# jianhengLiu/VINS-RGBD-FAST

Hardware: AMD Instinct MI355X
Metric: VIO frames/sec (640x480, 150 feats, 10-KF window) (higher is better)
Workload: dtype f64; 1 GPU; BASELINE configs[2]: 128 independent synthetic 640x480 RGB-D + 200 Hz IMU sequences per MI355X, 150 features, 10-keyframe window; sequences_per_gpu=128, tracker_lag=1, parallelism=sequences sharded per GPU, no data-path collective

## Files before the change

### vins-rgbd-fast_amd/csrc/be_kernels.hip

```cpp
#include <hip/hip_runtime.h>
#include "kernels.h"
#include "be_factors.h"

using namespace dm;

#if VIO_TIMERS
#define PH_INIT long long ph_t0 = (s == 0 && threadIdx.x == 0) ? VIO_CLOCK() : 0
#define PH(k) do { if (s == 0 && threadIdx.x == 0) { long long n_ = VIO_CLOCK(); B.timings[k] += (float)(n_ - ph_t0); ph_t0 = n_; } } while (0)
#else
#define PH_INIT do {} while (0)
#define PH(k) do {} while (0)
#endif

namespace {

struct Ctx {
    float *timings;
    const DevCfg *C;
    int s, W, P, LW, NL, NLs, NPR;
    BeSeq *be;
    FeSeq *fe;
    const vio_calibration *K;
    PreInt *pre;
    int *lm_id, *lm_start, *lm_nobs, *lm_est, *lm_solve, *lm_dyn, *lm_order, *lm_free, *lm_tmp, *lm_pidx, *lm_aidx, *lm_relo;
// ... 209 lines not shown
__device__ void lm_compact(Ctx &c, int *flags, int *offs, int *scratch) {
    int n = c.be->n_lm;
    int kept = block_scan_flags(flags, n, offs, scratch);
    const int t = threadIdx.x, nt = blockDim.x;
    int nfree0 = c.be->n_free;
    for (int k = t; k < n; k += nt) c.lm_tmp[k] = c.lm_order[k];
    __syncthreads();
    for (int k = t; k < n; k += nt) {
        int slot = c.lm_tmp[k];
        if (flags[k]) c.lm_order[offs[k]] = slot;
        else c.lm_free[nfree0 + (k - offs[k])] = slot;
    }
    __syncthreads();
    if (t == 0) { c.be->n_lm = kept; c.be->n_free = nfree0 + (n - kept); }
    __syncthreads();
}

}

__device__ m3 pnp_rodrigues(v3 r) {
    const double th = nrm(r);
    if (th < 2.220446049250313e-16) return eye();
    const v3 k = scl(1.0 / th, r);
    const double cth = cos(th), sth = sin(th), c1 = 1 - cth;
    const m3 K = skew(k);
    const double kk[3] = {k.x, k.y, k.z};
    m3 R;
    for (int i = 0; i < 3; i++) for (int j = 0; j < 3; j++) R.a[i * 3 + j] = (i == j ? cth : 0.0) + c1 * kk[i] * kk[j] + sth * K.a[i * 3 + j];
    return R;
}
// ... 1308 lines not shown
                be.initFirstPoseFlag = 0; be.prevTime = -1; be.n_lm = 0; be.n_free = c.NL; be.ring_base = 0;
                be.imu_head = be.imu_count_ingest;
                be.relo_info = 0;
                be.reboot_count++;
                be.status_code = VIO_REBOOTED;
                be.rebooted = 1;
                be.do_marg = 0;
                be.overflow = 0;
            }
        }
    }
}

}

template <bool EXACT> __device__ void marg_body(const Batch &B, int s, int *scratch, double *sred, unsigned char *smem_marg);
__device__ void finish_body(const Batch &B, int s, int *scratch, PreWork &pw, unsigned char *smem_marg);

__device__ __forceinline__ void solve_body(const Batch &B, int s, int *scratch, double *sred, unsigned char *smem, PreWork &pw);

__global__ __launch_bounds__(1024) void be_solve_kernel(Batch B) {
    const int s = blockIdx.x + B.s0;
    __shared__ int scratch[2 * 1024 + 8];
    __shared__ double sred[64];
    extern __shared__ __attribute__((aligned(16))) unsigned char smem[];
    PreWork &pw = *(PreWork *)(smem + 16 * ((B.cfg->LW * 8 + 15) / 16));
    solve_body(B, s, scratch, sred, smem, pw);
}
__global__ __launch_bounds__(512) void be_solve_kernel_512(Batch B) {
    const int s = blockIdx.x + B.s0;
    __shared__ int scratch[2 * 1024 + 8];
    __shared__ double sred[64];
    extern __shared__ __attribute__((aligned(16))) unsigned char smem[];
    PreWork &pw = *(PreWork *)(smem + 16 * ((B.cfg->LW * 8 + 15) / 16));
    solve_body(B, s, scratch, sred, smem, pw);
}
__global__ __launch_bounds__(512) void be_marg_kernel(Batch B) {
    const int s = blockIdx.x + B.s0;
    __shared__ int scratch[2 * 512 + 8];
    __shared__ double sred[64];
    __shared__ PreWork pw;
    extern __shared__ __attribute__((aligned(16))) unsigned char smem[];
    marg_body<false>(B, s, scratch, sred, smem);
    __syncthreads();
    finish_body(B, s, scratch, pw, smem);
}
__global__ __launch_bounds__(512) void be_marg_exact_kernel(Batch B) {
    const int s = blockIdx.x + B.s0;
    __shared__ int scratch[2 * 512 + 8];
    __shared__ double sred[64];
    __shared__ PreWork pw;
    extern __shared__ __attribute__((aligned(16))) unsigned char smem[];
    marg_body<true>(B, s, scratch, sred, smem);
    __syncthreads();
    finish_body(B, s, scratch, pw, smem);
}

__device__ __forceinline__ void solve_body(const Batch &B, int s, int *scratch, double *sred, unsigned char *smem, PreWork &pw) {
    const int t = threadIdx.x, nt = blockDim.x;
    Ctx c = make_ctx(B, s);
    const DevCfg &C = *B.cfg;
    const vio_config &cfg = C.c;
    BeSeq &be = *c.be;
    if (!be.do_solve) return;
    const int W = c.W, P = c.P, LW = c.LW, W1 = W + 1;
    __shared__ Params X, Xc;
    __shared__ double sdx[6 * VIO_MAXW + 16], srp[6 * VIO_MAXW + 16];
    __shared__ int sh_i[8];
    __shared__ double sh_d[8];
    double *xs = (double *)smem;
// ... 467 lines not shown
    }
    for (int i = t; i < n; i += nt) {
        double sacc = b[md + i];
        for (int k = 0; k < md; k++) sacc -= ET1[(size_t)i * m + k] * b[k];
        for (int k = md; k < m; k++) sacc -= ET1[(size_t)i * m + k] * c.gl[k - md];
        br[i] = sacc;
    }
    __syncthreads();
    if (VIO_TIMERS && t == 0) be.dbg[8] = (int)(VIO_CLOCK() - tx0);
    const int sw2 = marg_literal_prior(c, be, Ar, br, n, c.margW, A, sred, smem);
    if (VIO_TIMERS && t == 0) be.dbg[9] = (int)(VIO_CLOCK() - tx0);
    if (t == 0) { be.dbg[0] = sw1 * 100 + sw2; be.dbg[2] = second_new ? 1 : 0; be.dbg[4] = m; }
    if (VIO_TIMERS && t == 0) be.dbg[10] = (int)(VIO_CLOCK() - tx0);
}

template <bool EXACT> __device__ void marg_body(const Batch &B, int s, int *scratch, double *sred, unsigned char *smem_marg) {
    const int t = threadIdx.x, nt = blockDim.x;
    Ctx c = make_ctx(B, s);
    const DevCfg &C = *B.cfg;
    const vio_config &cfg = C.c;
    BeSeq &be = *c.be;
    if (!be.do_marg || be.rebooted || be.frame_count < c.W) return;
    const int W = c.W, W1 = W + 1, n = c.NPR;
    const double eps = 1e-8;
    __shared__ Params X;
    __shared__ double sdx[6 * VIO_MAXW + 16], srp[6 * VIO_MAXW + 16];
    __shared__ double cs[VIO_MAXW * 3 + 10], sn[VIO_MAXW * 3 + 10];
    __shared__ int pp[VIO_MAXW * 3 + 10], qq[VIO_MAXW * 3 + 10];
    __shared__ double A15[225], V15[225], Pinv[225];
    __shared__ int newpresent[VIO_MAXW + 3];
    const bool second_new = be.marginalization_flag != 0;
// ... 10 lines not shown
        quat q = R2q(ldm(be.Rs[i]));
        X.pose[i * 7 + 3] = q.x; X.pose[i * 7 + 4] = q.y; X.pose[i * 7 + 5] = q.z; X.pose[i * 7 + 6] = q.w;
        for (int k = 0; k < 3; k++) { X.sb[i * 9 + k] = be.Vs[i][k]; X.sb[i * 9 + 3 + k] = be.Bas[i][k]; X.sb[i * 9 + 6 + k] = be.Bgs[i][k]; }
    }
    if (t == W + 1) {
        X.ex[0] = be.tic[0]; X.ex[1] = be.tic[1]; X.ex[2] = be.tic[2];
        quat q = R2q(ldm(be.ric));
        X.ex[3] = q.x; X.ex[4] = q.y; X.ex[5] = q.z; X.ex[6] = q.w;
        X.td = be.td;
    }
    if (t < W + 3) newpresent[t] = 0;
    __syncthreads();
    if (t <= W) for (int k = 0; k < 7; k++) be.para_Pose[t][k] = X.pose[t * 7 + k];
    const int md = second_new ? 6 : 15;
    const int mq = md + n;
    double *A = c.margA, *b = c.margB;
    for (int i = t; i < mq * mq; i += nt) A[i] = 0;
    for (int i = t; i < mq; i += nt) b[i] = 0;
    __syncthreads();
    const int rS = md + 6 * W, rE = md + 6 * W + 9, rT = md + 6 * W + 15;
    if (be.has_prior) {
        prior_dx(c, X, sdx);
        for (int i = t; i < n; i += nt) {
            double sacc = c.prior_r[i];
            for (int j0 = 0; j0 < n; j0 += 32) {
                double hv[32];
#pragma unroll
                for (int u = 0; u < 32; u++) hv[u] = c.prior_H[(size_t)min(j0 + u, n - 1) * n + i];
#pragma unroll
                for (int u = 0; u < 32; u++) if (j0 + u < n) sacc += hv[u] * sdx[j0 + u];
            }
// ... 21 lines not shown
            }
        }
        for (int a = t; a < n; a += nt) b[pmap(a)] += srp[a];
        if (t < W + 3) {
            const int pres = be.prior_present[t];
            if (t > W) { if (pres) newpresent[t] = 1; }
            else if (second_new) { if (t < W - 1 || t == W) newpresent[t] = pres; }
            else if (t >= 1 && t < W && pres) newpresent[t - 1] = 1;
        }
        __syncthreads();
    }
    PH(16);
    if (!second_new) {
        PreInt &p1 = c.pre[be.pre_idx[1]];
        if (cfg.use_imu && bf::imu_marg_uses(p1)) {
            double *Jw = c.pairblk;
            double *raw = c.imu_raw;
            if ((t & 63) == 0) for (int part = t >> 6; part < 5; part += nt >> 6) {
                double unused = 0;
                bf::imu_work_item(p1, false, ld3(be.g), &X.pose[0], &X.sb[0], &X.pose[7], &X.sb[9], part, true, raw, unused);
            }
            __syncthreads();
            for (int w = t; w < 450; w += nt) {
                int r = w / 30, col = w - r * 30;
                double sacc = 0;
                for (int k = 0; k <= r; k++) sacc += p1.sqrt_info[r * 15 + k] * raw[k * 31 + col];
                Jw[w] = sacc;
            }
            __syncthreads();
            for (int w = t; w < 930; w += nt) {
                int a = w / 31, bb = w - a * 31;
// ... 110 lines not shown
                        int lm = min(kk, K - 1) >> 1, sub = kk & 1;
                        const double *Jr = c.res + (size_t)(lm * per + j - 1) * 42;
                        double v0 = Jr[sub * 20 + li];
                        double v1 = Jr[li < 3 ? sub * 20 + 16 + li : 40 + sub];
                        x0[u] = valid ? v0 : 0.0;
                        x1[u] = (valid && li < 4) ? v1 : 0.0;
                    }
#pragma unroll
                    for (int u = 0; u < 16; u++) {
                        if (k0 + 16 * (u >> 2) >= K) break;
                        a00 = __builtin_amdgcn_mfma_f64_16x16x4f64(x0[u], x0[u], a00, 0, 0, 0);
                        a10 = __builtin_amdgcn_mfma_f64_16x16x4f64(x1[u], x0[u], a10, 0, 0, 0);
                        a11 = __builtin_amdgcn_mfma_f64_16x16x4f64(x1[u], x1[u], a11, 0, 0, 0);
                    }
                }
                double *out = c.pairblk + (size_t)(j - 1) * 210;
#pragma unroll
                for (int r = 0; r < 4; r++) {
                    int row = lk + 4 * r, col = li;
                    if (col <= row) out[sym_idx(col, row)] = a00[r];
                    if (row < 4) out[sym_idx(col, 16 + row)] = a10[r];
                    if (row < 4 && col < 4 && col <= row) out[sym_idx(16 + col, 16 + row)] = a11[r];
                }
            }
        }
        if (!exact) for (int li = t; li < F0c; li += nt) { double d = c.Hll[li]; c.Hll[li] = d > eps ? 1.0 / d : 0.0; }
        __syncthreads();
        PH(24);
        __shared__ signed char qfr[6 * VIO_MAXW + 40], qlc[6 * VIO_MAXW + 40];
        __shared__ double sub_part[4][6 * VIO_MAXW + 40];
        for (int a = t; a <= mq; a += nt) {
// ... 15 lines not shown
        for (int w0 = t; w0 < mq * (mq + 1); w0 += 4 * nt) {
            bool use[4], multi[4], rhs[4];
            int dst[4], row[4], sidx[4];
            double pv[4], av[4];
#pragma unroll
            for (int u = 0; u < 4; u++) {
                const int w = min(w0 + u * nt, mq * (mq + 1) - 1);
                const int a = w / (mq + 1), bb = w - a * (mq + 1);
                const int fa = qfr[a], fb = qfr[bb];
                const int la = qlc[a], lb = qlc[bb];
                use[u] = w0 + u * nt < mq * (mq + 1) && fa >= 0 && fb >= 0 && !(fa > 0 && fb > 0 && fa != fb);
                multi[u] = use[u] && fa == 0 && fb == 0;
                rhs[u] = bb == mq; row[u] = a; dst[u] = a * mq + bb;
                sidx[u] = sym_idx(la, lb);
                const int f1 = fa > 0 ? fa : (fb > 0 ? fb : 1);
                pv[u] = use[u] ? c.pairblk[(size_t)(f1 - 1) * 210 + sidx[u]] : 0.0;
                av[u] = use[u] ? (rhs[u] ? b[a] : A[dst[u]]) : 0.0;
            }
#pragma unroll
            for (int u = 0; u < 4; u++) {
                if (!use[u]) continue;
                double sacc = pv[u];
                if (multi[u]) {
                    double fv[VIO_MAXW];
#pragma unroll
                    for (int j = 0; j < VIO_MAXW; j++) fv[j] = c.pairblk[(size_t)min(j, W - 1) * 210 + sidx[u]];
                    sacc = 0;
#pragma unroll
                    for (int j = 0; j < VIO_MAXW; j++) if (j < W) sacc += fv[j];
                }
                if (!rhs[u]) A[dst[u]] = av[u] + sacc;
                else b[row[u]] = av[u] + (sacc - ((sub_part[0][row[u]] + sub_part[1][row[u]]) + (sub_part[2][row[u]] + sub_part[3][row[u]])));
            }
        }
        __syncthreads();
        PH(25);
        if (!exact) {
            const int lane = t & 63, wave = t >> 6, nw = nt >> 6, li = lane & 15, lk = lane >> 4;
            const int nbq = (mq + 15) >> 4, ntile = nbq * (nbq + 1) / 2;
            for (int tile = wave; tile < ntile; tile += nw) {
                int ti, tj;
// ... 59 lines not shown
        __syncthreads();
    }
    if (VIO_TIMERS && s == 0 && t == 0 && pinv_direct) B.timings[26] += 1.0f;
    PH(36);
    double *T1 = (double *)smem_marg, *Amr = T1 + (size_t)n * md;
    for (int w = t; w < n * md; w += nt) {
        int i = w / md, j = w - i * md;
        double sacc = 0;
        for (int k = 0; k < md; k++) sacc += A[(md + i) * mq + k] * Pinv[k * md + j];
        T1[w] = sacc;
        const int k2 = w / n, j2 = w - k2 * n;
        Amr[w] = A[k2 * mq + md + j2];
    }
    __syncthreads();
    PH(37);
    double *Ar = c.margV;
    double *br = c.vec;
    for (int w0 = t; w0 < n * n; w0 += 8 * nt) {
        double av[8];
#pragma unroll
        for (int u = 0; u < 8; u++) { const int w = min(w0 + u * nt, n * n - 1), i = w / n, j = w - i * n; av[u] = A[(md + i) * mq + md + j]; }
#pragma unroll
        for (int u = 0; u < 8; u++) {
            const int w = w0 + u * nt;
            if (w >= n * n) break;
            const int i = w / n, j = w - i * n;
            double tt = av[u];
            for (int k = 0; k < md; k++) tt -= T1[i * md + k] * Amr[k * n + j];
            Ar[w] = tt;
        }
    }
    for (int i = t; i < n; i += nt) {
        double sacc = b[md + i];
        for (int k = 0; k < md; k++) sacc -= T1[i * md + k] * b[k];
        br[i] = sacc;
    }
    __syncthreads();
    PH(21);
    if (lit2) {
        __shared__ int cert_bad;
        if (t == 0) cert_bad = pinv_direct ? 0 : 1;
        __syncthreads();
        double n_t = 0, n_d = 0, n_db = 0;
        if (!second_new) {
// ... 19 lines not shown
        n_s = block_sum(n_s, sred);
        __syncthreads();
        if (t == 0) {
            const double bound = sqrt(n_s) + 2.0 * sqrt(n_t) + sqrt(n_d) + sqrt(n_db) * sqrt(n_t);
            const bool certified = !cert_bad && isfinite(bound) && bound > 0.0 && 1.0 / bound > 1e-7;
            be.dbg[11] = certified ? 1 : 0;
            if (!certified) be.dbg[12] += 1;
        }
        __syncthreads();
        const int sw2 = marg_literal_prior(c, be, Ar, br, n, c.margW, A, sred, smem_marg);
        if (t == 0) { be.dbg[0] = sw2; be.dbg[2] = second_new ? 1 : 0; be.dbg[4] = md; }
    } else {
    for (int w0 = t; w0 < n * n; w0 += 8 * nt) {
        double x[8], y[8];
#pragma unroll
        for (int u = 0; u < 8; u++) { const int w = min(w0 + u * nt, n * n - 1), i = w / n, j = w - i * n; x[u] = Ar[i * n + j]; y[u] = Ar[j * n + i]; }
#pragma unroll
        for (int u = 0; u < 8; u++) if (w0 + u * nt < n * n) c.prior_H[w0 + u * nt] = 0.5 * (x[u] + y[u]);
    }
    for (int i = t; i < n; i += nt) c.prior_r[i] = br[i];
    PH(38);
    {
        __shared__ __attribute__((aligned(16))) double cq_x[EIG_LD + 16];
        __shared__ double cq_dinv[EIG_LD + 16];
        __shared__ int cq_flag;
        const int nbq = (n + 15) >> 4;
        double *T = (double *)smem_marg;
        double dmax = 0;
        for (int i = t; i < n; i += nt) dmax = fmax(dmax, fabs(Ar[i * n + i]));
        dmax = block_max(dmax, sred);
        const double delta = 64.0 * 2.220446049250313e-16 * (double)n * dmax;
        const int ntl = nbq * (nbq + 1) / 2 * 256;
        for (int w0 = t; w0 < ntl; w0 += 4 * nt) {
            double x[4], y[4];
            int ii[4], jj[4], dd[4];
#pragma unroll
            for (int u = 0; u < 4; u++) {
                const int w = min(w0 + u * nt, ntl - 1);
                int tile = w >> 8, e = w & 255, r = e >> 4, cc = e & 15, ti, tj;
                tri_decode(tile, ti, tj);
                const int i = 16 * ti + r, j = 16 * tj + cc, ic = min(i, n - 1), jc = min(j, n - 1);
                ii[u] = i; jj[u] = j; dd[u] = tl_idx(ti, tj, r, cc);
                x[u] = Ar[ic * n + jc]; y[u] = Ar[jc * n + ic];
            }
#pragma unroll
            for (int u = 0; u < 4; u++) {
                if (w0 + u * nt >= ntl) break;
                const int i = ii[u], j = jj[u];
                T[dd[u]] = (i < n && j < n) ? 0.5 * (x[u] + y[u]) + (i == j ? delta : 0.0) : (i == j ? 1.0 : 0.0);
            }
        }
        for (int i = t; i < 16 * nbq; i += nt) cq_x[i] = i < n ? br[i] : 0.0;
        __syncthreads();
        PH(39);
        double c0 = 0;
        if (dmax > 0 && chol_tiles(T, nbq, &cq_flag, cq_dinv, nullptr, cq_x)) {
            double acc = 0;
            for (int i = t; i < n; i += nt) acc += cq_x[i] * cq_x[i];
// ... 73 lines not shown
    for (int w = t; w < n * n; w += nt) {
        int k = w / n, i = w - k * n;
        double wv = ev_d[k];
        double S = wv > eps ? wv : 0.0;
        c.prior_J[w] = sqrt(S) * Vv[i * ldj + k];
    }
    for (int k = t; k < n; k += nt) {
        double wv = ev_d[k];
        double Sinv = wv > eps ? 1.0 / wv : 0.0;
        double vb = 0;
        for (int i = 0; i < n; i++) vb += Vv[i * ldj + k] * br[i];
        c.prior_rf[k] = sqrt(Sinv) * vb;
    }
}

__device__ void finish_body(const Batch &B, int s, int *scratch, PreWork &pw, unsigned char *smem_marg) {
    const int t = threadIdx.x, nt = blockDim.x;
    Ctx c = make_ctx(B, s);
    const DevCfg &C = *B.cfg;
    const vio_config &cfg = C.c;
    BeSeq &be = *c.be;
    const int W = c.W, W1 = W + 1;
    __shared__ int sh_i[4];
    double *od = B.odom + (size_t)s * 11;
    if (!be.processed || be.rebooted) return;
    PH_INIT;
    int nlm = be.n_lm;
    int *flag = c.lm_pidx, *offs = c.lm_aidx;
    const int fc = be.frame_count;
    const int sflag0 = be.solver_flag;
    __syncthreads();
    const bool dyn_initial = sflag0 == 0 && (cfg.dynamic_init || (fc == W && !be.do_solve && be.ex_pending));
    if (dyn_initial) {
        if (fc < W) {
            if (t == 0) be.frame_count = fc + 1;
            return;
        }
    } else if (sflag0 == 0) {
        if (fc == W && be.do_solve) {
            if (t == 0) be.solver_flag = 1;
            __syncthreads();
        } else {
            if (t == 0 && fc < W) {
                int n = fc + 1;
                for (int k = 0; k < 3; k++) { be.Ps[n][k] = be.Ps[fc][k]; be.Vs[n][k] = be.Vs[fc][k]; be.Bas[n][k] = be.Bas[fc][k]; be.Bgs[n][k] = be.Bgs[fc][k]; }
                for (int k = 0; k < 9; k++) be.Rs[n][k] = be.Rs[fc][k];
                be.frame_count = n;
            }
            return;
        }
    } else if (!be.init_frame) {
        m3 ric = ldm(be.ric);
        v3 tic = ld3(be.tic);
        for (int k = t; k < nlm; k += nt) {
            int slot = c.lm_order[k];
            if (!(c.lm_nobs[slot] >= 2 && c.lm_start[slot] < W - 2)) continue;
            double depth = c.lm_depth[slot];
            if (depth < 0) continue;
            int imu_i = c.lm_start[slot], no = c.lm_nobs[slot];
            const double *oi = obs_ptr(c, slot, imu_i);
            v3 pts_i = mk(oi[0], oi[1], oi[2]);
            double err = 0, err3 = 0;
            int cnt = 0;
            for (int q = 1; q < no; q++) {
                int imu_j = imu_i + q;
                const double *oj = obs_ptr(c, slot, imu_j);
                v3 pts_j = mk(oj[0], oj[1], oj[2]);
                v3 pts_w = add(mul(ldm(be.Rs[imu_i]), add(mul(ric, scl(depth, pts_i)), tic)), ld3(be.Ps[imu_i]));
                v3 pts_cj = mul(tr(ric), sub(mul(tr(ldm(be.Rs[imu_j])), sub(pts_w, ld3(be.Ps[imu_j]))), tic));
                double rx = pts_cj.x / pts_cj.z - pts_j.x, ry = pts_cj.y / pts_cj.z - pts_j.y;
                err += sqrt(rx * rx + ry * ry);
                err3 += nrm(sub(pts_cj, pts_j)) / depth;
                cnt++;
            }
// ... 9 lines not shown
            int first = be.pre_idx[0];
            for (int i = 0; i < W; i++) {
                be.Headers[i] = be.Headers[i + 1];
                for (int k = 0; k < 3; k++) { be.Ps[i][k] = be.Ps[i + 1][k]; be.Vs[i][k] = be.Vs[i + 1][k]; be.Bas[i][k] = be.Bas[i + 1][k]; be.Bgs[i][k] = be.Bgs[i + 1][k]; }
                for (int k = 0; k < 9; k++) be.Rs[i][k] = be.Rs[i + 1][k];
                be.pre_idx[i] = be.pre_idx[i + 1];
            }
            be.pre_idx[W] = first;
            bf::preint_init(c.pre[first], ld3(be.acc_0), ld3(be.gyr_0), ld3(be.Bas[W]), ld3(be.Bgs[W]));
        }
        __syncthreads();
        PH(28);
        m3 R0 = mul(ldm(be.back_R0), ldm(be.ric)), R1 = mul(ldm(be.Rs[0]), ldm(be.ric));
        v3 P0 = add(ld3(be.back_P0), mul(ldm(be.back_R0), ld3(be.tic))), P1 = add(ld3(be.Ps[0]), mul(ldm(be.Rs[0]), ld3(be.tic)));
        for (int k = t; k < nlm; k += nt) {
            int slot = c.lm_order[k];
            int keep = 1;
            if (c.lm_start[slot] != 0) c.lm_start[slot]--;
            else {
                const double *o0 = obs_ptr(c, slot, 0);
                v3 uv_i = mk(o0[0], o0[1], o0[2]);
                int no = c.lm_nobs[slot] - 1;
                c.lm_nobs[slot] = no;
                if (dyn_initial) keep = no > 0;
                else if (no < 2) keep = 0;
                else {
                    v3 pts_i = scl(c.lm_depth[slot], uv_i);
                    v3 w_pts_i = add(mul(R0, pts_i), P0);
                    v3 pts_j = mul(tr(R1), sub(w_pts_i, P1));
                    c.lm_depth[slot] = pts_j.z > 0 ? pts_j.z : cfg.init_depth;
                }
            }
            flag[k] = keep;
        }
        __syncthreads();
        if (t == 0) be.ring_base = (be.ring_base + 1) % W1;
        __syncthreads();
        lm_compact(c, flag, offs, scratch);
    } else {
        PreInt &dst = c.pre[be.pre_idx[W - 1]];
        PreInt &src = c.pre[be.pre_idx[W]];
        if (t == 0) {
            be.Headers[W - 1] = be.Headers[W];
            for (int k = 0; k < 3; k++) { be.Ps[W - 1][k] = be.Ps[W][k]; be.Vs[W - 1][k] = be.Vs[W][k]; be.Bas[W - 1][k] = be.Bas[W][k]; be.Bgs[W - 1][k] = be.Bgs[W][k]; }
            for (int k = 0; k < 9; k++) be.Rs[W - 1][k] = be.Rs[W][k];
        }
        preint_load(dst, pw);
        PreintNoSide none;
        preint_propagate_many<false>(dst, pw, *c.K, src.n_buf, PreintArrays{src.dt_buf, src.acc_buf, src.gyr_buf}, none, true, (double *)smem_marg);
        preint_store(dst, pw);
        if (t == 0) bf::preint_init(src, ld3(be.acc_0), ld3(be.gyr_0), ld3(be.Bas[W]), ld3(be.Bgs[W]));
        __syncthreads();
        for (int k = t; k < nlm; k += nt) {
            int slot = c.lm_order[k];
            int keep = 1;
            int st = c.lm_start[slot], no = c.lm_nobs[slot];
            if (st == W) {
                double *d = obs_ptr(c, slot, W - 1);
                const double *sr = obs_ptr(c, slot, W);
                for (int q = 0; q < VIO_OBS_D; q++) d[q] = sr[q];
                c.lm_start[slot] = st - 1;
            } else {
                int endf = st + no - 1;
                if (endf >= W - 1) {
                    if (endf == W) {
                        double *d = obs_ptr(c, slot, W - 1);
                        const double *sr = obs_ptr(c, slot, W);
                        for (int q = 0; q < VIO_OBS_D; q++) d[q] = sr[q];
                    }
                    c.lm_nobs[slot] = no - 1;
                    if (no - 1 == 0) keep = 0;
                }
            }
            flag[k] = keep;
        }
        __syncthreads();
        lm_compact(c, flag, offs, scratch);
    }
    PH(29);
    if (dyn_initial) {
        if (t == 0 && (be.overflow & ~VIO_OVF_DEVIATION)) be.overflow_frames++;
        return;
    }
    if (sflag0 == 1) {
        nlm = be.n_lm;
        for (int k = t; k < nlm; k += nt) flag[k] = c.lm_solve[c.lm_order[k]] == 2 ? 0 : 1;
        __syncthreads();
        lm_compact(c, flag, offs, scratch);
    }
    if (t == 0) {
        for (int k = 0; k < 9; k++) { be.last_R[k] = be.Rs[W][k]; be.last_R0[k] = be.Rs[0][k]; }
        for (int k = 0; k < 3; k++) { be.last_P[k] = be.Ps[W][k]; be.last_P0[k] = be.Ps[0][k]; }
        quat q = R2q(ldm(be.Rs[W]));
        od[0] = be.Headers[W];
        od[1] = be.Ps[W][0]; od[2] = be.Ps[W][1]; od[3] = be.Ps[W][2];
        od[4] = q.w; od[5] = q.x; od[6] = q.y; od[7] = q.z;
        od[8] = be.Vs[W][0]; od[9] = be.Vs[W][1]; od[10] = be.Vs[W][2];
        int hc = B.odom_count[s];
        double *hrow = B.odom_hist + ((size_t)s * B.hist_cap + (hc % B.hist_cap)) * 11;
        for (int k = 0; k < 11; k++) hrow[k] = od[k];
        B.odom_count[s] = hc + 1;
        if (be.overflow & ~VIO_OVF_DEVIATION) be.overflow_frames++;
    }
    PH(30);
// ... 240 lines not shown
```

### vins-rgbd-fast_amd/csrc/kernels.h

```cpp
#pragma once
#include <hip/hip_runtime.h>
#include "vio_state.h"
#include "../../include/vio_synth.h"

#define PI_CH 8
#define PREINT_MANY_LDS_DOUBLES (PI_CH * (225 + 270))
static inline size_t fast_lds_bytes(int rw, int rh) {
    return (size_t)(((rw + 6) * rh + 15) & ~15) + (size_t)((rw * rh + 15) & ~15) + (size_t)(((rw - 6) * (rh - 6) + 63) / 64 + 2) * 8 + 16;
}
__host__ __device__ static inline size_t ps_eval_lds_bytes(int W) {
    const size_t W1 = (size_t)W + 1, a = (W1 * W1 + 1) * 32 * 8, b = (size_t)W * (VIO_PREINT_HDR + 1) * 8;
    return (a > b ? a : b) + 64;
}
static inline size_t ps_ls_lds_bytes(int W) { (void)W; return ((((sizeof(Params) / sizeof(double)) + 1) & ~(size_t)1) + 176) * 8 + 16; }
struct LkImages {
    const uint8_t *prev[4];
    const uint8_t *next[4];
    int w[4], h[4];
};

__global__ void fe_begin_kernel(Batch B, const double *stamps, int gate, int publish, const uint8_t *modes, const double *R_rel);
__global__ void be_latest_odometry_kernel(Batch B, int seq, double *out11);
__global__ void be_imu_rate_odometry_kernel(Batch B, const double *since, int cap, int *n_rows, double *rows, double *last);
__global__ void fe_predict_motion_kernel(Batch B, int seq, double t0, double t1, double *out9);
// ... 12 lines not shown
__global__ void fe_fast_kernel(Batch B);
__global__ void fe_fast_stage_kernel(const uint8_t *img, int W, GridRect r, uint32_t *out, int cap, int *count);
__global__ void fe_add_kernel(Batch B, int gate);
struct IngestSrc {
    const int *n_obs;
    const int *ids;
    const double *obs;
    const double *stamps;
    int cap;
};
template <bool EXCALIB> __global__ void be_ingest_kernel(Batch B, const uint16_t *depth_base, size_t depth_stride, IngestSrc src);
__global__ void be_stage_relative_r_kernel(int n, const double *corres6, double *R9, int *detail8);
__global__ void be_solve_kernel(Batch B);
__global__ void be_solve_kernel_512(Batch B);
__global__ void be_marg_kernel(Batch B);
__global__ void be_marg_exact_kernel(Batch B);
__global__ void ps_setup_kernel(Batch B);
__global__ void ps_eval_kernel(Batch B);
__global__ void ps_eval_kernel_occ3(Batch B);
__global__ void ps_eval_kernel_occ4(Batch B);
__global__ void ps_asm_a_kernel(Batch B);
__global__ void ps_asm_a_kernel_occ4(Batch B);
__global__ void ps_asm_b_schur_kernel(Batch B, int nb_b, int by_blocks);
__global__ void ps_serial_big_kernel(Batch B);
__global__ void ps_serial_kernel_512(Batch B);
__global__ void ps_final_kernel(Batch B);
__global__ void ps_ls_kernel(Batch B);
__global__ void ps_evalf_kernel(Batch B);
static inline size_t ps_evalf_lds_bytes(int W) {
    const size_t W1 = (size_t)W + 1, a = ((size_t)PS_FUSE_CAP * 28 + (W1 * W / 2 + 1) * 32) * 8 + (size_t)PS_FUSE_CAP * 12, b = ((size_t)W * (VIO_PREINT_HDR + 1) + (size_t)W * 465) * 8;
// ... 33 lines not shown
```

### vins-rgbd-fast_amd/csrc/vio_abi.hip

```cpp
#include "vio_handle.h"

thread_local std::string g_err;

namespace {

void circle_halfwidths(int radius, int *hw) {
    for (int i = 0; i <= radius; i++) hw[i] = -1;
    int err = 0, dx = radius, dy = 0, plus = 1, minus = (radius << 1) - 1;
    while (dx >= dy) {
        if (dx > hw[dy]) hw[dy] = dx;
        if (dy > hw[dx]) hw[dx] = dy;
        dy++;
        err += plus;
        plus += 2;
        int mask = (err <= 0) - 1;
        err -= minus & mask;
        dx += mask;
        minus -= mask & 2;
    }
}

}

static size_t ingest_lds_bytes(const DevCfg &C, bool excalib) {
// ... 473 lines not shown
            HIPCHK(hipGraphLaunch(g.solve_graph, st));
        } else
            launch_phased();
    } else if (be_threads <= 512) be_solve_kernel_512<<<S, be_threads, h->lds_solve, st>>>(Bg);
    else be_solve_kernel<<<S, be_threads, h->lds_solve, st>>>(Bg);
    if (prof) PEV(h, 10);
    (void)hipEventRecord(g.ev_solve, st);
    g.have_solve_ev = true;
    if (C.c.dynamic_init && one_seq < 0 && &g == &h->groups.back()) {
        state_gather_kernel<<<(h->S + 255) / 256, 256, 0, st>>>(h->B, h->d_state);
        HIPCHK(hipMemcpyAsync(h->h_state, h->d_state, sizeof(int) * h->S, hipMemcpyDeviceToHost, st));
        HIPCHK(hipEventRecord(h->ev_state, st));
        h->state_pending = true;
    }
    if (C.MX > 0) be_marg_exact_kernel<<<S, h->marg_threads, h->lds_marg, st>>>(Bg);
    else be_marg_kernel<<<S, h->marg_threads, h->lds_marg, st>>>(Bg);
    if (prof) PEV(h, 11);
    HIPCHK(hipGetLastError());
    return VIO_OK;
}

}

namespace vio_internal {
int refresh_dynamic_state(vio_batch *h) {
    if (!h->hc.c.dynamic_init) return VIO_OK;
    if (h->state_pending) {
        HIPCHK(hipEventSynchronize(h->ev_state));
        h->state_pending = false;
        bool any = false;
        for (int s = 0; s < h->S; s++) {
// ... 174 lines not shown
static void read_knobs(vio_batch *h) {
    h->be_threads = std::min(1024, std::max(64, env_int("VIO_BE_THREADS", h->be_threads) & ~63));
    h->asm_b_by_blocks = std::max(0, std::min(2, env_int("VIO_ASM_B_MODE", h->asm_b_by_blocks)));
    h->ps_asm_b_blocks = h->hc.W <= 10 ? 12 : 24;
    h->ps_asm_b_blocks = std::max(1, std::min(256, env_int("VIO_ASM_B_BLOCKS", h->ps_asm_b_blocks)));
    h->eval_occ = env_int("VIO_EVAL_OCC", h->eval_occ);
    h->use_graph = env_int("VIO_GRAPH", h->use_graph) != 0;
    h->xcd_map = env_int("VIO_XCD_MAP", h->xcd_map);
    h->fe_xcd_map = env_int("VIO_FE_XCD_MAP", h->fe_xcd_map);
    h->xcd_n = env_int("VIO_XCD_N", h->xcd_n);
    h->feed_throttle = env_int("VIO_FEED_THROTTLE", h->feed_throttle) != 0;
    h->uploads_in_flight = env_int("VIO_UPLOADS_IN_FLIGHT", h->uploads_in_flight) == 1 ? 1 : 2;
    h->extra_slots = std::max(1, env_int("VIO_EXTRA_SLOTS", h->extra_slots));
    h->asm_a_occ4 = env_int("VIO_ASM_A_OCC", 0) >= 4;
    h->marg_threads = std::min(512, std::max(64, env_int("VIO_MARG_THREADS", h->marg_threads) & ~63));
    h->B.flags = env_int("VIO_FLAGS", 0);
}

static int create_groups(vio_batch *h) {
    const DevCfg &C = h->hc;
    const int n_seq = h->S;
    int per = env_int("VIO_GROUP_SEQS", n_seq);
    if (per < 1) per = 1;
    if (C.c.dynamic_init) per = n_seq;
    int ng = (n_seq + per - 1) / per;
    if (ng > 16) { ng = 16; per = (n_seq + ng - 1) / ng; ng = (n_seq + per - 1) / per; }
    h->groups.resize(ng);
    for (int k = 0; k < ng; k++) {
        vio_batch::Group &g = h->groups[k];
        g.s0 = k * per;
// ... 63 lines not shown
            int nact = 0;
            for (size_t a = 0; a < nb; a++) for (size_t b2 = 0; b2 <= a; b2++) {
                auto act = [&](size_t cb) { const size_t c0 = 16 * cb, c1 = c0 + 15; return c0 < 6 * W1 || (c1 >= 15 * W1 && c0 < 15 * W1 + 7); };
                if (act(a) && act(b2)) nact++;
            }
            h->ps_schur_tiles = nact;
            h->B.n_schur = nact;
            h->B.gn_ext = env_int("VIO_GN_EXT", 1) != 0;
        }
    }
    {
        size_t nbq = ((size_t)C.NPRIOR + 15) >> 4;
        h->lds_marg = std::max(std::max((size_t)nbq * (nbq + 1) / 2 * 2048, (size_t)2 * C.NPRIOR * 15 * 8), (size_t)PREINT_MANY_LDS_DOUBLES * 8) + 64;
        if (C.MXL > 0) h->lds_marg = std::max(h->lds_marg, marg_exact_lds_bytes(C.MXL));
        if (C.MX > 0) h->lds_marg = std::max(h->lds_marg, (size_t)7 * 512 * 8 + 64);
        h->lds_factor = C.NPRIOR <= 96 ? (size_t)C.NPRIOR * (C.NPRIOR | 1) * 8 + 64 : 64;
        (void)raise_lds_limit((const void *)be_prior_factor_kernel, h->lds_factor);
    }
    (void)raise_lds_limit((const void *)be_marg_kernel, (size_t)(h->lds_marg));
    (void)raise_lds_limit((const void *)be_marg_exact_kernel, (size_t)(h->lds_marg));
    const bool excalib = C.c.estimate_extrinsic == 2;
    const void *ingest = excalib ? (const void *)be_ingest_kernel<true> : (const void *)be_ingest_kernel<false>;
    (void)raise_lds_limit(ingest, ingest_lds_bytes(C, excalib));

    (void)raise_lds_limit((const void *)fe_select_kernel, (size_t)(h->lds_select));
    (void)raise_lds_limit((const void *)fe_add_kernel, (size_t)(h->lds_add));
    (void)raise_lds_limit((const void *)fe_fast_kernel, (size_t)(h->lds_fast));
    bool fits = lds_fits(C.MX > 0 ? (const void *)be_marg_exact_kernel : (const void *)be_marg_kernel, h->lds_marg, "be_marg") &&
                lds_fits(ingest, ingest_lds_bytes(C, excalib), "be_ingest") &&
                lds_fits((const void *)fe_select_kernel, h->lds_select, "fe_select") && lds_fits((const void *)fe_add_kernel, h->lds_add, "fe_add") &&
                lds_fits((const void *)fe_fast_kernel, h->lds_fast, "fe_fast");
    if (fits && h->solve_mode == 1)
        fits = lds_fits((const void *)ps_eval_kernel, h->lds_ps_eval, "ps_eval") && lds_fits((const void *)ps_ls_kernel, h->lds_ps_ls, "ps_ls") &&
               lds_fits(h->serial_big ? (const void *)ps_serial_big_kernel : (const void *)ps_serial_kernel_512, h->lds_serial, "ps_serial");
    else if (fits)
        fits = lds_fits(h->be_threads <= 512 ? (const void *)be_solve_kernel_512 : (const void *)be_solve_kernel, h->lds_solve, "be_solve");
    return fits ? VIO_OK : VIO_ECAPACITY;
}

static int handle_init(vio_batch *h, int n_seq) {
    size_marg_exact(h);
    h->S = n_seq;
    const DevCfg &C = h->hc;
// ... 467 lines not shown
```

### vins-rgbd-fast_amd/csrc/vio_handle.h

```cpp
#pragma once
#include <hip/hip_runtime.h>
#include <limits.h>
#include <math.h>
#include <algorithm>
#include <cmath>
#include <stdlib.h>
#include <mutex>
#include <chrono>
#include <string>
#include <string.h>
#include <vector>
#include "kernels.h"
#include "dyninit_host.h"
#include "camera_model.h"
#include "snapshot.h"
#include "stage_util.h"

struct vio_batch {
    DevCfg hc;
    Batch B;
    int S;
    int device = -1;
    struct Group {
        int s0 = 0, n = 0;
// ... 73 lines not shown
        double *h_t = nullptr, *h_acc = nullptr, *h_gyr = nullptr, *d_t = nullptr, *d_acc = nullptr, *d_gyr = nullptr;
        size_t cap = 0;
        hipEvent_t done = nullptr;
        bool busy = false;
    } imu_stage[2];
    int imu_stage_cur = 0;
    hipEvent_t ev_imu = nullptr;
    std::vector<double> last_imu_t;
    size_t lds_select = 0, lds_add = 0, lds_fast = 0, lds_solve = 0, lds_serial = 0, lds_marg = 0, lds_factor = 0, lds_ps_ls = 0, lds_ps_evalf = 0;
    int ps_evalf_blocks = 0;
    bool feed_throttle = true;
    int uploads_in_flight = 2;
    int relo_frames = 0;
    bool line_search = true;
    int be_threads = 512, marg_threads = 384;
    int solve_mode = 1;
    bool asm_a_occ4 = false;
    int eval_occ = 0;
    bool serial_big = false;
    size_t lds_ps_eval = 0;
    int ps_eval_blocks = 0, ps_asm_a_blocks = 0, ps_schur_tiles = 0;
    bool timing_valid = false;
    std::vector<hipEvent_t> pev;
    int prof_steps = 0, prof_cur = -1;
    bool prof_fe_only = false;
    struct SnapRow { const char *name; int kind; unsigned char *base; int64_t bytes, blob_off; };
    std::vector<SnapRow> snap_rows;
    int64_t snap_dev_bytes = 0, snap_chunks = 0;
    int snap_entries = 0;
    SnapEntry *d_snap_tab = nullptr;
// ... 235 lines not shown
```

Before: 60420 frames/s.

## Keep marginalisation system and landmark tables resident in LDS

Adds an LDS-resident variant of the marginalisation kernel that places the dense prior system A/b, the Schur-reduced block and the per-frame Jacobian blocks in shared memory instead of global scratch. It also stages landmark order, start and nobs tables in LDS during the finish phase, and compacts them there before writing back. The aim is to cut global-memory round trips in a latency-bound per-sequence block. The cost is a much larger LDS footprint, which may lower occupancy. The old global path stays as a fallback kernel, selected when the LDS request does not fit or an env flag disables it.

```diff
diff --git a/vins-rgbd-fast_amd/csrc/be_kernels.hip b/vins-rgbd-fast_amd/csrc/be_kernels.hip
--- a/vins-rgbd-fast_amd/csrc/be_kernels.hip
+++ b/vins-rgbd-fast_amd/csrc/be_kernels.hip
@@ -247,6 +247,18 @@
     __syncthreads();
     if (t == 0) { c.be->n_lm = kept; c.be->n_free = nfree0 + (n - kept); }
     __syncthreads();
+}
+
+__device__ void lm_compact_staged(Ctx &c, int *ord, int *tmp, int *flags, int *offs, int *scratch, int &n, int &nfree) {
+    const int kept = block_scan_flags(flags, n, offs, scratch);
+    const int t = threadIdx.x, nt = blockDim.x;
+    for (int k = t; k < n; k += nt) tmp[k] = ord[k];
+    __syncthreads();
+    for (int k = t; k < n; k += nt) if (flags[k]) ord[offs[k]] = tmp[k];
+    for (int k = t; k < n; k += nt) if (!flags[k]) c.lm_free[nfree + (k - offs[k])] = tmp[k];
+    __syncthreads();
+    nfree += n - kept;
+    n = kept;
 }
 
 }
@@ -1585,8 +1597,8 @@
 
 }
 
-template <bool EXACT> __device__ void marg_body(const Batch &B, int s, int *scratch, double *sred, unsigned char *smem_marg);
-__device__ void finish_body(const Batch &B, int s, int *scratch, PreWork &pw, unsigned char *smem_marg);
+template <bool EXACT, bool LDSA> __device__ void marg_body(const Batch &B, int s, int *scratch, double *sred, unsigned char *smem_marg);
+template <bool LT> __device__ void finish_body(const Batch &B, int s, int *scratch, PreWork &pw, unsigned char *smem_marg);
 
 __device__ __forceinline__ void solve_body(const Batch &B, int s, int *scratch, double *sred, unsigned char *smem, PreWork &pw);
 
@@ -1612,9 +1624,19 @@
     __shared__ double sred[64];
     __shared__ PreWork pw;
     extern __shared__ __attribute__((aligned(16))) unsigned char smem[];
-    marg_body<false>(B, s, scratch, sred, smem);
-    __syncthreads();
-    finish_body(B, s, scratch, pw, smem);
+    marg_body<false, true>(B, s, scratch, sred, smem);
+    __syncthreads();
+    finish_body<true>(B, s, scratch, pw, smem);
+}
+__global__ __launch_bounds__(512) void be_marg_hbm_kernel(Batch B) {
+    const int s = blockIdx.x + B.s0;
+    __shared__ int scratch[2 * 512 + 8];
+    __shared__ double sred[64];
+    __shared__ PreWork pw;
+    extern __shared__ __attribute__((aligned(16))) unsigned char smem[];
+    marg_body<false, false>(B, s, scratch, sred, smem);
+    __syncthreads();
+    finish_body<false>(B, s, scratch, pw, smem);
 }
 __global__ __launch_bounds__(512) void be_marg_exact_kernel(Batch B) {
     const int s = blockIdx.x + B.s0;
@@ -1622,9 +1644,9 @@
     __shared__ double sred[64];
     __shared__ PreWork pw;
     extern __shared__ __attribute__((aligned(16))) unsigned char smem[];
-    marg_body<true>(B, s, scratch, sred, smem);
-    __syncthreads();
-    finish_body(B, s, scratch, pw, smem);
+    marg_body<true, false>(B, s, scratch, sred, smem);
+    __syncthreads();
+    finish_body<false>(B, s, scratch, pw, smem);
 }
 
 __device__ __forceinline__ void solve_body(const Batch &B, int s, int *scratch, double *sred, unsigned char *smem, PreWork &pw) {
@@ -2122,7 +2144,8 @@
     if (VIO_TIMERS && t == 0) be.dbg[10] = (int)(VIO_CLOCK() - tx0);
 }
 
-template <bool EXACT> __device__ void marg_body(const Batch &B, int s, int *scratch, double *sred, unsigned char *smem_marg) {
+template <bool EXACT, bool LDSA> __device__ void marg_body(const Batch &B, int s, int *scratch, double *sred, unsigned char *smem_marg) {
+    static_assert(!(EXACT && LDSA), "the literal marginalisation keeps its system in HBM");
     const int t = threadIdx.x, nt = blockDim.x;
     Ctx c = make_ctx(B, s);
     const DevCfg &C = *B.cfg;
@@ -2163,7 +2186,10 @@
     if (t <= W) for (int k = 0; k < 7; k++) be.para_Pose[t][k] = X.pose[t * 7 + k];
     const int md = second_new ? 6 : 15;
     const int mq = md + n;
-    double *A = c.margA, *b = c.margB;
+    double *const ovl = (double *)smem_marg;
+    double *const Ares = (double *)(smem_marg + marg_overlay_bytes(n, W, true));
+    double *A = LDSA ? Ares : c.margA, *b = LDSA ? Ares + (size_t)(n + 15) * (n + 15) : c.margB;
+    double *Gj = LDSA ? ovl : c.pairblk;
     for (int i = t; i < mq * mq; i += nt) A[i] = 0;
     for (int i = t; i < mq; i += nt) b[i] = 0;
     __syncthreads();
@@ -2215,7 +2241,7 @@
     if (!second_new) {
         PreInt &p1 = c.pre[be.pre_idx[1]];
         if (cfg.use_imu && bf::imu_marg_uses(p1)) {
-            double *Jw = c.pairblk;
+            double *Jw = Gj;
             double *raw = c.imu_raw;
             if ((t & 63) == 0) for (int part = t >> 6; part < 5; part += nt >> 6) {
                 double unused = 0;
@@ -2356,7 +2382,7 @@
                         a11 = __builtin_amdgcn_mfma_f64_16x16x4f64(x1[u], x1[u], a11, 0, 0, 0);
                     }
                 }
-                double *out = c.pairblk + (size_t)(j - 1) * 210;
+                double *out = Gj + (size_t)(j - 1) * 210;
 #pragma unroll
                 for (int r = 0; r < 4; r++) {
                     int row = lk + 4 * r, col = li;
@@ -2402,7 +2428,7 @@
                 rhs[u] = bb == mq; row[u] = a; dst[u] = a * mq + bb;
                 sidx[u] = sym_idx(la, lb);
                 const int f1 = fa > 0 ? fa : (fb > 0 ? fb : 1);
-                pv[u] = use[u] ? c.pairblk[(size_t)(f1 - 1) * 210 + sidx[u]] : 0.0;
+                pv[u] = use[u] ? Gj[(size_t)(f1 - 1) * 210 + sidx[u]] : 0.0;
                 av[u] = use[u] ? (rhs[u] ? b[a] : A[dst[u]]) : 0.0;
             }
 #pragma unroll
@@ -2412,7 +2438,7 @@
                 if (multi[u]) {
                     double fv[VIO_MAXW];
 #pragma unroll
-                    for (int j = 0; j < VIO_MAXW; j++) fv[j] = c.pairblk[(size_t)min(j, W - 1) * 210 + sidx[u]];
+                    for (int j = 0; j < VIO_MAXW; j++) fv[j] = Gj[(size_t)min(j, W - 1) * 210 + sidx[u]];
                     sacc = 0;
 #pragma unroll
                     for (int j = 0; j < VIO_MAXW; j++) if (j < W) sacc += fv[j];
@@ -2502,8 +2528,9 @@
     }
     __syncthreads();
     PH(37);
-    double *Ar = c.margV;
-    double *br = c.vec;
+    const int lda = LDSA ? mq : n;
+    double *Ar = LDSA ? A + (size_t)md * mq + md : c.margV;
+    double *br = LDSA ? Ares + (size_t)(n + 15) * (n + 16) : c.vec;
     for (int w0 = t; w0 < n * n; w0 += 8 * nt) {
         double av[8];
 #pragma unroll
@@ -2515,7 +2542,7 @@
             const int i = w / n, j = w - i * n;
             double tt = av[u];
             for (int k = 0; k < md; k++) tt -= T1[i * md + k] * Amr[k * n + j];
-            Ar[w] = tt;
+            Ar[i * lda + j] = tt;
         }
     }
     for (int i = t; i < n; i += nt) {
@@ -2565,7 +2592,7 @@
     for (int w0 = t; w0 < n * n; w0 += 8 * nt) {
         double x[8], y[8];
 #pragma unroll
-        for (int u = 0; u < 8; u++) { const int w = min(w0 + u * nt, n * n - 1), i = w / n, j = w - i * n; x[u] = Ar[i * n + j]; y[u] = Ar[j * n + i]; }
+        for (int u = 0; u < 8; u++) { const int w = min(w0 + u * nt, n * n - 1), i = w / n, j = w - i * n; x[u] = Ar[i * lda + j]; y[u] = Ar[j * lda + i]; }
 #pragma unroll
         for (int u = 0; u < 8; u++) if (w0 + u * nt < n * n) c.prior_H[w0 + u * nt] = 0.5 * (x[u] + y[u]);
     }
@@ -2578,7 +2605,7 @@
         const int nbq = (n + 15) >> 4;
         double *T = (double *)smem_marg;
         double dmax = 0;
-        for (int i = t; i < n; i += nt) dmax = fmax(dmax, fabs(Ar[i * n + i]));
+        for (int i = t; i < n; i += nt) dmax = fmax(dmax, fabs(Ar[i * lda + i]));
         dmax = block_max(dmax, sred);
         const double delta = 64.0 * 2.220446049250313e-16 * (double)n * dmax;
         const int ntl = nbq * (nbq + 1) / 2 * 256;
@@ -2592,7 +2619,7 @@
                 tri_decode(tile, ti, tj);
                 const int i = 16 * ti + r, j = 16 * tj + cc, ic = min(i, n - 1), jc = min(j, n - 1);
                 ii[u] = i; jj[u] = j; dd[u] = tl_idx(ti, tj, r, cc);
-                x[u] = Ar[ic * n + jc]; y[u] = Ar[jc * n + ic];
+                x[u] = Ar[ic * lda + jc]; y[u] = Ar[jc * lda + ic];
             }
 #pragma unroll
             for (int u = 0; u < 4; u++) {
@@ -2696,7 +2723,7 @@
     }
 }
 
-__device__ void finish_body(const Batch &B, int s, int *scratch, PreWork &pw, unsigned char *smem_marg) {
+template <bool LT> __device__ void finish_body(const Batch &B, int s, int *scratch, PreWork &pw, unsigned char *smem_marg) {
     const int t = threadIdx.x, nt = blockDim.x;
     Ctx c = make_ctx(B, s);
     const DevCfg &C = *B.cfg;
@@ -2708,7 +2735,20 @@
     if (!be.processed || be.rebooted) return;
     PH_INIT;
     int nlm = be.n_lm;
-    int *flag = c.lm_pidx, *offs = c.lm_aidx;
+    int *const tab = (int *)(smem_marg + marg_overlay_bytes(c.NPR, W, true));
+    int *const flag = LT ? tab + 2 * c.NL : c.lm_pidx, *const offs = LT ? tab + 3 * c.NL : c.lm_aidx;
+    int *const ord = LT ? tab : c.lm_order, *const otmp = tab + c.NL, *const lst = tab + 4 * c.NL, *const lno = tab + 5 * c.NL;
+    const int nlm0 = nlm;
+    int nfree = be.n_free;
+    if (LT) for (int k = t; k < nlm; k += nt) { const int slot = c.lm_order[k]; ord[k] = slot; lst[k] = c.lm_start[slot]; lno[k] = c.lm_nobs[slot]; }
+    auto lm_st = [&](int k, int slot) -> int { return LT ? lst[k] : c.lm_start[slot]; };
+    auto lm_no = [&](int k, int slot) -> int { return LT ? lno[k] : c.lm_nobs[slot]; };
+    auto compact = [&]() { if (LT) lm_compact_staged(c, ord, otmp, flag, offs, scratch, nlm, nfree); else lm_compact(c, flag, offs, scratch); };
+    auto stage_back = [&]() {
+        if (!LT) return;
+        for (int k = t; k < nlm0; k += nt) { c.lm_order[k] = ord[k]; c.lm_pidx[k] = flag[k]; c.lm_aidx[k] = offs[k]; }
+        if (t == 0) { be.n_lm = nlm; be.n_free = nfree; }
+    };
     const int fc = be.frame_count;
     const int sflag0 = be.solver_flag;
     __syncthreads();
@@ -2735,11 +2775,11 @@
         m3 ric = ldm(be.ric);
         v3 tic = ld3(be.tic);
         for (int k = t; k < nlm; k += nt) {
-            int slot = c.lm_order[k];
-            if (!(c.lm_nobs[slot] >= 2 && c.lm_start[slot] < W - 2)) continue;
+            int slot = ord[k];
+            const int imu_i = lm_st(k, slot), no = lm_no(k, slot);
+            if (!(no >= 2 && imu_i < W - 2)) continue;
             double depth = c.lm_depth[slot];
             if (depth < 0) continue;
-            int imu_i = c.lm_start[slot], no = c.lm_nobs[slot];
             const double *oi = obs_ptr(c, slot, imu_i);
             v3 pts_i = mk(oi[0], oi[1], oi[2]);
             double err = 0, err3 = 0;
@@ -2779,13 +2819,14 @@
         m3 R0 = mul(ldm(be.back_R0), ldm(be.ric)), R1 = mul(ldm(be.Rs[0]), ldm(be.ric));
         v3 P0 = add(ld3(be.back_P0), mul(ldm(be.back_R0), ld3(be.tic))), P1 = add(ld3(be.Ps[0]), mul(ldm(be.Rs[0]), ld3(be.tic)));
         for (int k = t; k < nlm; k += nt) {
-            int slot = c.lm_order[k];
+            int slot = ord[k];
             int keep = 1;
-            if (c.lm_start[slot] != 0) c.lm_start[slot]--;
+            const int st = lm_st(k, slot);
+            if (st != 0) c.lm_start[slot] = st - 1;
             else {
                 const double *o0 = obs_ptr(c, slot, 0);
                 v3 uv_i = mk(o0[0], o0[1], o0[2]);
-                int no = c.lm_nobs[slot] - 1;
+                int no = lm_no(k, slot) - 1;
                 c.lm_nobs[slot] = no;
                 if (dyn_initial) keep = no > 0;
                 else if (no < 2) keep = 0;
@@ -2801,7 +2842,7 @@
         __syncthreads();
         if (t == 0) be.ring_base = (be.ring_base + 1) % W1;
         __syncthreads();
-        lm_compact(c, flag, offs, scratch);
+        compact();
     } else {
         PreInt &dst = c.pre[be.pre_idx[W - 1]];
         PreInt &src = c.pre[be.pre_idx[W]];
@@ -2817,9 +2858,9 @@
         if (t == 0) bf::preint_init(src, ld3(be.acc_0), ld3(be.gyr_0), ld3(be.Bas[W]), ld3(be.Bgs[W]));
         __syncthreads();
         for (int k = t; k < nlm; k += nt) {
-            int slot = c.lm_order[k];
+            int slot = ord[k];
             int keep = 1;
-            int st = c.lm_start[slot], no = c.lm_nobs[slot];
+            int st = lm_st(k, slot), no = lm_no(k, slot);
             if (st == W) {
                 double *d = obs_ptr(c, slot, W - 1);
                 const double *sr = obs_ptr(c, slot, W);
@@ -2840,19 +2881,21 @@
             flag[k] = keep;
         }
         __syncthreads();
-        lm_compact(c, flag, offs, scratch);
+        compact();
     }
     PH(29);
     if (dyn_initial) {
         if (t == 0 && (be.overflow & ~VIO_OVF_DEVIATION)) be.overflow_frames++;
+        stage_back();
         return;
     }
     if (sflag0 == 1) {
-        nlm = be.n_lm;
-        for (int k = t; k < nlm; k += nt) flag[k] = c.lm_solve[c.lm_order[k]] == 2 ? 0 : 1;
-        __syncthreads();
-        lm_compact(c, flag, offs, scratch);
-    }
+        if (!LT) nlm = be.n_lm;
+        for (int k = t; k < nlm; k += nt) flag[k] = c.lm_solve[ord[k]] == 2 ? 0 : 1;
+        __syncthreads();
+        compact();
+    }
+    stage_back();
     if (t == 0) {
         for (int k = 0; k < 9; k++) { be.last_R[k] = be.Rs[W][k]; be.last_R0[k] = be.Rs[0][k]; }
         for (int k = 0; k < 3; k++) { be.last_P[k] = be.Ps[W][k]; be.last_P0[k] = be.Ps[0][k]; }
diff --git a/vins-rgbd-fast_amd/csrc/kernels.h b/vins-rgbd-fast_amd/csrc/kernels.h
--- a/vins-rgbd-fast_amd/csrc/kernels.h
+++ b/vins-rgbd-fast_amd/csrc/kernels.h
@@ -5,6 +5,16 @@
 
 #define PI_CH 8
 #define PREINT_MANY_LDS_DOUBLES (PI_CH * (225 + 270))
+__host__ __device__ static inline size_t marg_overlay_bytes(int nprior, int W, bool gj) {
+    const size_t nbq = ((size_t)nprior + 15) >> 4, tiles = nbq * (nbq + 1) / 2 * 2048, t1 = (size_t)2 * nprior * 15 * 8, pi = (size_t)PREINT_MANY_LDS_DOUBLES * 8;
+    size_t m = tiles > t1 ? tiles : t1;
+    m = m > pi ? m : pi;
+    if (gj && (size_t)W * 210 * 8 > m) m = (size_t)W * 210 * 8;
+    return ((m + 15) & ~(size_t)15) + 64;
+}
+#define MARG_LM_TABLES 6
+__host__ __device__ static inline size_t marg_resident_doubles(int nprior) { const size_t q = (size_t)nprior + 15; return q * q + q + (size_t)nprior; }
+__host__ __device__ static inline size_t marg_resident_lds_bytes(int nprior, int W) { return marg_overlay_bytes(nprior, W, true) + marg_resident_doubles(nprior) * 8; }
 static inline size_t fast_lds_bytes(int rw, int rh) {
     return (size_t)(((rw + 6) * rh + 15) & ~15) + (size_t)((rw * rh + 15) & ~15) + (size_t)(((rw - 6) * (rh - 6) + 63) / 64 + 2) * 8 + 16;
 }
@@ -50,6 +60,7 @@
 __global__ void be_solve_kernel(Batch B);
 __global__ void be_solve_kernel_512(Batch B);
 __global__ void be_marg_kernel(Batch B);
+__global__ void be_marg_hbm_kernel(Batch B);
 __global__ void be_marg_exact_kernel(Batch B);
 __global__ void ps_setup_kernel(Batch B);
 __global__ void ps_eval_kernel(Batch B);
diff --git a/vins-rgbd-fast_amd/csrc/vio_abi.hip b/vins-rgbd-fast_amd/csrc/vio_abi.hip
--- a/vins-rgbd-fast_amd/csrc/vio_abi.hip
+++ b/vins-rgbd-fast_amd/csrc/vio_abi.hip
@@ -511,7 +511,8 @@
         h->state_pending = true;
     }
     if (C.MX > 0) be_marg_exact_kernel<<<S, h->marg_threads, h->lds_marg, st>>>(Bg);
-    else be_marg_kernel<<<S, h->marg_threads, h->lds_marg, st>>>(Bg);
+    else if (h->marg_lds) be_marg_kernel<<<S, h->marg_threads, h->lds_marg, st>>>(Bg);
+    else be_marg_hbm_kernel<<<S, h->marg_threads, h->lds_marg, st>>>(Bg);
     if (prof) PEV(h, 11);
     HIPCHK(hipGetLastError());
     return VIO_OK;
@@ -716,6 +717,7 @@
     h->extra_slots = std::max(1, env_int("VIO_EXTRA_SLOTS", h->extra_slots));
     h->asm_a_occ4 = env_int("VIO_ASM_A_OCC", 0) >= 4;
     h->marg_threads = std::min(512, std::max(64, env_int("VIO_MARG_THREADS", h->marg_threads) & ~63));
+    h->marg_lds = env_int("VIO_MARG_LDS", 1) != 0;
     h->B.flags = env_int("VIO_FLAGS", 0);
 }
 
@@ -809,11 +811,21 @@
         h->lds_marg = std::max(std::max((size_t)nbq * (nbq + 1) / 2 * 2048, (size_t)2 * C.NPRIOR * 15 * 8), (size_t)PREINT_MANY_LDS_DOUBLES * 8) + 64;
         if (C.MXL > 0) h->lds_marg = std::max(h->lds_marg, marg_exact_lds_bytes(C.MXL));
         if (C.MX > 0) h->lds_marg = std::max(h->lds_marg, (size_t)7 * 512 * 8 + 64);
+        {
+            hipFuncAttributes fa;
+            int cap = 0;
+            if (hipDeviceGetAttribute(&cap, hipDeviceAttributeMaxSharedMemoryPerBlock, h->device) != hipSuccess || cap <= 0) cap = 160 * 1024;
+            const size_t want = marg_resident_lds_bytes(C.NPRIOR, C.W);
+            h->marg_lds = h->marg_lds && C.MX == 0 && (size_t)MARG_LM_TABLES * C.NL * 4 <= marg_resident_doubles(C.NPRIOR) * 8 &&
+                          hipFuncGetAttributes(&fa, (const void *)be_marg_kernel) == hipSuccess && fa.sharedSizeBytes + want <= (size_t)cap;
+            if (h->marg_lds) h->lds_marg = want;
+        }
         h->lds_factor = C.NPRIOR <= 96 ? (size_t)C.NPRIOR * (C.NPRIOR | 1) * 8 + 64 : 64;
         (void)raise_lds_limit((const void *)be_prior_factor_kernel, h->lds_factor);
     }
     (void)raise_lds_limit((const void *)be_marg_kernel, (size_t)(h->lds_marg));
     (void)raise_lds_limit((const void *)be_marg_exact_kernel, (size_t)(h->lds_marg));
+    (void)raise_lds_limit((const void *)be_marg_hbm_kernel, (size_t)(h->lds_marg));
     const bool excalib = C.c.estimate_extrinsic == 2;
     const void *ingest = excalib ? (const void *)be_ingest_kernel<true> : (const void *)be_ingest_kernel<false>;
     (void)raise_lds_limit(ingest, ingest_lds_bytes(C, excalib));
@@ -821,7 +833,7 @@
     (void)raise_lds_limit((const void *)fe_select_kernel, (size_t)(h->lds_select));
     (void)raise_lds_limit((const void *)fe_add_kernel, (size_t)(h->lds_add));
     (void)raise_lds_limit((const void *)fe_fast_kernel, (size_t)(h->lds_fast));
-    bool fits = lds_fits(C.MX > 0 ? (const void *)be_marg_exact_kernel : (const void *)be_marg_kernel, h->lds_marg, "be_marg") &&
+    bool fits = lds_fits(C.MX > 0 ? (const void *)be_marg_exact_kernel : h->marg_lds ? (const void *)be_marg_kernel : (const void *)be_marg_hbm_kernel, h->lds_marg, "be_marg") &&
                 lds_fits(ingest, ingest_lds_bytes(C, excalib), "be_ingest") &&
                 lds_fits((const void *)fe_select_kernel, h->lds_select, "fe_select") && lds_fits((const void *)fe_add_kernel, h->lds_add, "fe_add") &&
                 lds_fits((const void *)fe_fast_kernel, h->lds_fast, "fe_fast");
diff --git a/vins-rgbd-fast_amd/csrc/vio_handle.h b/vins-rgbd-fast_amd/csrc/vio_handle.h
--- a/vins-rgbd-fast_amd/csrc/vio_handle.h
+++ b/vins-rgbd-fast_amd/csrc/vio_handle.h
@@ -111,6 +111,7 @@
     int relo_frames = 0;
     bool line_search = true;
     int be_threads = 512, marg_threads = 384;
+    bool marg_lds = true;
     int solve_mode = 1;
     bool asm_a_occ4 = false;
     int eval_occ = 0;
```

Result: faster. 61220 frames/s, median of 6 (+1.3%).
